# xinpw8/pokegym

Hardware: AMD Instinct MI355X
Metric: aggregate env.step/sec (higher is better)
Workload: dtype u8

## Files before the change

pokegym_amd/csrc/pk_capi.cpp:

```cpp
#include <hip/hip_runtime.h>

#include <errno.h>
#include <stdarg.h>
#include <stdio.h>
#include <stdlib.h>
#include <string.h>

#include <string>
#include <vector>

#include "../../include/pokegym_amd.h"
#include "pk_ucode.h"
#include "pk_layout.h"
#include "pk_reward.h"

hipError_t pk_launch_step(const PkStepArgs& a, hipStream_t s);
hipError_t pk_launch_step_small(const PkStepArgs& a, hipStream_t s);
hipError_t pk_launch_render(const PkStepArgs& a, hipStream_t s);
hipError_t pk_launch_reset(const PkResetArgs& a, hipStream_t s);
hipError_t pk_launch_list(const uint8_t* mask, uint32_t env0, uint32_t env1, uint32_t* cnt, uint32_t* ids, hipStream_t s);
hipError_t pk_launch_render_latched(const PkStepArgs& a, hipStream_t s);
hipError_t pk_launch_gather_env(const uint8_t* mem, uint32_t env, uint32_t sh, uint8_t* out, hipStream_t s);
hipError_t pk_launch_gather_range(const uint8_t* mem, uint32_t env0, uint32_t count, uint32_t sh, uint8_t* out, hipStream_t s);
hipError_t pk_launch_scatter_env(uint8_t* mem, uint32_t env, uint32_t sh, const uint8_t* in, hipStream_t s);
hipError_t pk_launch_done(const uint32_t* time_reg, uint32_t n, uint32_t max_steps, uint8_t* term,
                          uint8_t* trunc, double* rew, hipStream_t s);
hipError_t pk_launch_reward(const PkRewardArgs& a, hipStream_t s);
hipError_t pk_launch_rreset_pre(const PkRewardArgs& a, hipStream_t s);
hipError_t pk_launch_rreset_post(const PkRewardArgs& a, hipStream_t s);
hipError_t pk_launch_obs(const PkRewardArgs& a, hipStream_t s);
hipError_t pk_launch_seen_rehash(const uint32_t* old_tab, uint32_t old_lg, uint32_t* new_tab, uint32_t new_lg,
                                 const uint32_t* rs, uint32_t n, uint32_t np, hipStream_t s);
hipError_t pk_launch_ram_copy(uint8_t* mem, uint8_t* dense, uint32_t n, uint32_t sh, uint32_t phys0, uint32_t len,
                              uint32_t to_dense, hipStream_t s);
hipError_t pk_launch_bank_list(const PkBankArgs& a, hipStream_t s);
hipError_t pk_launch_bank_copy(const PkBankArgs& a, hipStream_t s);
hipError_t pk_launch_ep_move(const PkEpArgs& a, hipStream_t s);
hipError_t pk_launch_arch_update(const PkArchArgs& a, hipStream_t s);
hipError_t pk_launch_arch_draw(const PkArchArgs& a, hipStream_t s);
hipError_t pk_launch_arch_merge(const PkArchArgs& a, hipStream_t s);
hipError_t pk_launch_xchg_pack(const PkPackArgs& p, hipStream_t s);
hipError_t pk_launch_xchg_move(const PkXchgArgs& x, bool pack, hipStream_t s);
hipError_t pk_launch_arch_out(const PkArchArgs& a, hipStream_t s);
hipError_t pk_launch_cell_keys(const uint8_t* mem, uint32_t sh, uint32_t shift, uint64_t* keys, uint32_t env0,
                               uint32_t env1, hipStream_t s);
hipError_t pk_launch_frame_keys(const PkCellArgs& a, hipStream_t s);
hipError_t pk_launch_fstack(const PkStackArgs& a, hipStream_t s);
hipError_t pk_launch_cnt_update(const PkCountArgs& a, hipStream_t s);
hipError_t pk_launch_cnt_add(const PkCountArgs& a, hipStream_t s);
hipError_t pk_launch_cnt_pack(const PkCountArgs& a, hipStream_t s);
hipError_t pk_launch_traj_record(const PkTrajArgs& a, hipStream_t s);
hipError_t pk_launch_traj_reset(const PkTrajArgs& a, hipStream_t s);
hipError_t pk_launch_traj_mark(const PkTrajArgs& a, hipStream_t s);
hipError_t pk_launch_traj_move(const PkTrajArgs& a, hipStream_t s);
hipError_t pk_launch_traj_get(const PkTrajArgs& a, hipStream_t s);

namespace {

thread_local std::string g_err;

int fail(int code, const char* fmt, ...) {
    char buf[512];
    va_list ap;
    va_start(ap, fmt);
    vsnprintf(buf, sizeof buf, fmt, ap);
    va_end(ap);
    g_err = buf;
    return code;
}

#define HIPCHK(expr)                                                                       \
    do {                                                                                   \
        hipError_t e_ = (expr);                                                            \
        if (e_ != hipSuccess) return fail(-EIO, "%s: %s", #expr, hipGetErrorString(e_)); \
    } while (0)

constexpr size_t S_VER = 0, S_HDR = 1, S_CPU = 5, S_VRAM = 23, S_OAM = 8215, S_LCDREG = 8375,
                 S_LCDX = 8386, S_CLOCK = 8388, S_TARGET = 8396, S_NEXTMODE = 8404,
                 S_SCAN = 8405, S_SCREEN = 9125, S_WRAM = 101285, S_FEA0 = 109477,
                 S_IO = 109573, S_HRAM = 109649, S_FF4C = 109776, S_TIMER = 109828,
                 S_MBC = 109836, S_SRAM = 109842, S_SIZE = 142610;

struct Template {
    uint32_t regs[PK_NREGS];
    std::vector<uint8_t> mem;
    uint32_t lat[3 * PK_ROWS];
    std::vector<uint8_t> screen;
    uint8_t hdr[4];
    uint8_t lcdx[2];
};

uint64_t rd64(const uint8_t* p) {
    uint64_t v = 0;
    for (int i = 7; i >= 0; i--) v = (v << 8) | p[i];
    return v;
}
void wr64(uint8_t* p, uint64_t v) {
    for (int i = 0; i < 8; i++) { p[i] = (uint8_t)v; v >>= 8; }
}

int parse_v9(const uint8_t* s, size_t len, Template& t) {
// ... 608 lines not shown
    if (wram && (addr & 0x1FFF) + len > 0x2000) return fail(-EINVAL, "pk_set_ram: range wraps the echo mirror");
    HIPCHK(hipSetDevice(h->device));
    uint32_t phys0 = wram ? PK_P_WRAM + (addr & 0x1FFFu) : PK_P_HRAM + (addr - 0xFF80u);
    HIPCHK(pk_launch_ram_copy(h->mem, const_cast<uint8_t*>(dense), h->n, h->ilv_sh, phys0, len, 0, (hipStream_t)stream));
    return traj_mark(h, nullptr, nullptr, 0, h->n, (hipStream_t)stream);
}

static uint32_t k1_wave_lanes(const pk_handle* h, uint32_t count) {
    if (h->wave_lanes) return h->wave_lanes;
    const uint32_t npad = (count + PK_LANES - 1u) & ~(PK_LANES - 1u);
    if (npad / 64u >= 2u * h->simds) return 64u;
    if (npad / 32u >= 2u * h->simds) return 32u;
    if (npad / 16u > h->simds && npad / 16u <= 2u * h->simds) return 16u;
    return 32u;
}

static void k1_shape(const pk_handle* h, bool small, uint32_t& lanes, uint32_t& block, uint32_t& prio) {
    lanes = k1_wave_lanes(h, h->n);
    const uint32_t wg_envs = small ? PK_SMALL_WG_ENVS : PK_WG_ENVS;
    const uint32_t max_threads = small ? PK_SMALL_MAX_THREADS : PK_K1_MAX_THREADS;
    if (h->k1_block) {
        block = h->k1_block < max_threads ? h->k1_block : max_threads;
        if ((block / PK_LANES) * lanes > wg_envs) block = wg_envs / lanes * PK_LANES;
    } else {
        const uint32_t waves = ((h->n + PK_LANES - 1u) / PK_LANES) * (PK_LANES / lanes);
        const uint32_t wide = wg_envs * PK_LANES / lanes < max_threads ? wg_envs * PK_LANES / lanes : max_threads;
        block = waves <= h->simds ? 256u : wide;
    }
    prio = h->k1_prio >= 0 ? (uint32_t)h->k1_prio : (block > 256u && !small ? 1u : 0u);
}

static bool k1_small(const pk_handle* h, uint32_t env0, uint32_t env1) {
    if (h->k1_small >= 0) return h->k1_small != 0 && k1_wave_lanes(h, h->n) <= 32u;
    return (env1 - env0) < h->n && k1_wave_lanes(h, h->n) <= 32u;
}

static PkStepArgs step_args(pk_handle* h, const uint8_t* actions, uint32_t env0, uint32_t env1) {
    PkStepArgs a;
    memset(&a, 0, sizeof a);
    a.mem = h->mem; a.rom = h->rom; a.romw = reinterpret_cast<const uint32_t*>(h->rom); a.regs = h->regs; a.ucode = h->ucode; a.actions = actions;
    a.lat = h->lat; a.screen = h->screen; a.n = h->n; a.npad = h->npad;
    a.rom_bank_mask = h->bank_mask; a.mbc = h->mbc; a.frames = h->frames;
    a.release_frame = h->release; a.render_last = (h->flags & PK_F_RENDER) ? 1 : 0;
    a.lat_stride = (uint32_t)h->lat_stride;
    const bool small = k1_small(h, env0, env1);
    a.small = small ? 1u : 0u;
    a.nslots = small ? h->nslots_s : h->nslots;
    a.bank_slot = small ? h->bank_slot_s : h->bank_slot;
    a.slot_bank = small ? h->slot_bank_s : h->slot_bank;
    a.all_staged = a.nslots >= h->bank_mask + 1u ? 1u : 0u;
    k1_shape(h, small, a.wave_lanes, a.block, a.prio);
    a.simds = h->simds;
    a.dbg = h->dbg;
    a.env0 = env0; a.env1 = env1;
    a.ilv_sh = h->ilv_sh;
    return a;
}

int pk_render_latched(pk_handle* h, void* stream) {
    if (!h) return fail(-EINVAL, "null handle");
    HIPCHK(hipSetDevice(h->device));
    PkStepArgs a = step_args(h, nullptr, 0, h->n);
    HIPCHK(pk_launch_render_latched(a, (hipStream_t)stream));
    return 0;
}

int pk_step_range(pk_handle* h, uint32_t env0, uint32_t count, const uint8_t* actions, double* rew, uint8_t* term,
                  uint8_t* trunc, void* stream) {
    int rc;
    if ((rc = check_range(h, env0, count))) return rc;
    if (!actions) return fail(-EINVAL, "actions_dev is required");
    HIPCHK(hipSetDevice(h->device));
    hipStream_t s = (hipStream_t)stream;
    const uint32_t env1 = env0 + count;
    PkStepArgs a = step_args(h, actions, env0, env1);
    if (h->prof && (rc = prof_event(h, s))) return rc;
    HIPCHK(a.small ? pk_launch_step_small(a, s) : pk_launch_step(a, s));
    if (h->traj_cap) {
        PkTrajArgs t = traj_args(h, env0, env1);
        t.actions = actions;
        HIPCHK(pk_launch_traj_record(t, s));
    }
    if (h->prof && (rc = prof_event(h, s))) return rc;
    if (a.render_last) HIPCHK(pk_launch_render(a, s));
    if (h->prof && (rc = prof_event(h, s))) return rc;
    if (h->flags & PK_F_REWARD) {
        PkRewardArgs r = reward_args(h, env0, env1);
        r.actions = actions; r.rew = rew; r.term = term; r.trunc = trunc;
        HIPCHK(pk_launch_reward(r, s));
        HIPCHK(pk_launch_obs(r, s));
    } else if (rew || term || trunc) {
        HIPCHK(pk_launch_done(h->regs + (size_t)PK_R_TIME * h->npad + env0, count, h->max_steps, term ? term + env0 : nullptr,
                              trunc ? trunc + env0 : nullptr, rew ? rew + env0 : nullptr, s));
    }
    if (h->prof && (rc = prof_event(h, s))) return rc;
    return 0;
}

int pk_step(pk_handle* h, const uint8_t* actions, uint8_t* screen_out, double* rew, uint8_t* term,
            uint8_t* trunc, void* stream) {
    if (!h) return fail(-EINVAL, "null handle");
    int rc = pk_step_range(h, 0, h->n, actions, rew, term, trunc, stream);
    if (rc) return rc;
    if (screen_out)
        HIPCHK(hipMemcpyAsync(screen_out, h->screen, (size_t)h->n * PK_SCREEN, hipMemcpyDeviceToDevice, (hipStream_t)stream));
    return 0;
}

static int fetch_env(pk_handle* h, uint32_t env, std::vector<uint8_t>& mem, uint32_t* regs,
                     uint32_t* lat, std::vector<uint8_t>& screen) {
    if (env >= h->n) return fail(-EINVAL, "env %u out of range (n=%u)", env, h->n);
    HIPCHK(hipSetDevice(h->device));
    HIPCHK(hipDeviceSynchronize());
    HIPCHK(pk_launch_gather_env(h->mem, env, h->ilv_sh, h->scratch, nullptr));
    mem.resize(PK_PHYS);
    HIPCHK(hipMemcpy(mem.data(), h->scratch, PK_PHYS, hipMemcpyDeviceToHost));
    for (uint32_t f = 0; f < PK_NREGS; f++)
        HIPCHK(hipMemcpy(&regs[f], h->regs + (size_t)f * h->npad + env, 4, hipMemcpyDeviceToHost));
    uint32_t gid = env / PK_LANES, lane = env % PK_LANES;
    for (uint32_t k = 0; k < 3; k++) {
        std::vector<uint32_t> tmp((size_t)PK_ROWS * PK_LANES);
        HIPCHK(hipMemcpy(tmp.data(), h->lat + k * h->lat_stride + (size_t)gid * PK_ROWS * PK_LANES,
                         tmp.size() * 4, hipMemcpyDeviceToHost));
        for (uint32_t y = 0; y < PK_ROWS; y++) lat[k * PK_ROWS + y] = tmp[(size_t)y * PK_LANES + lane];
    }
    screen.resize(PK_SCREEN);
    HIPCHK(hipMemcpy(screen.data(), h->screen + (size_t)env * PK_SCREEN, PK_SCREEN, hipMemcpyDeviceToHost));
    return 0;
}

int pk_snapshot(pk_handle* h, uint32_t env, uint8_t* out, uint64_t len) {
    if (!h || !out) return fail(-EINVAL, "null argument");
    if (len < S_SIZE) return fail(-EINVAL, "buffer too small for a v9 state");
    std::vector<uint8_t> mem, screen;
    uint32_t regs[PK_NREGS], lat[3 * PK_ROWS];
    int rc = fetch_env(h, env, mem, regs, lat, screen);
    if (rc) return rc;
    export_v9(h->tmpl, regs, mem.data(), lat, screen.data(), out);
    return 0;
}

int pk_snapshot_range(pk_handle* h, uint32_t env0, uint32_t count, uint8_t* out, uint64_t len) {
    if (!h || !out) return fail(-EINVAL, "null argument");
    if (count == 0) return 0;
    if ((uint64_t)env0 + count > h->n) return fail(-EINVAL, "envs [%u, %u) out of range (n=%u)", env0, env0 + count, h->n);
    if (len < (uint64_t)count * S_SIZE) return fail(-EINVAL, "buffer too small for %u v9 states", count);
    HIPCHK(hipSetDevice(h->device));
    HIPCHK(hipDeviceSynchronize());
    const uint32_t chunk = count < 1024u ? count : 1024u;
    uint8_t* dmem = nullptr;
    HIPCHK(hipMalloc((void**)&dmem, (size_t)chunk * PK_PHYS));
    std::vector<uint8_t> mem((size_t)chunk * PK_PHYS), screen((size_t)chunk * PK_SCREEN);
    std::vector<uint32_t> regs((size_t)PK_NREGS * chunk), latg;
    int rc = 0;
    for (uint32_t c0 = 0; c0 < count && !rc; c0 += chunk) {
        const uint32_t e0 = env0 + c0, m = (count - c0) < chunk ? (count - c0) : chunk;
        hipError_t e = pk_launch_gather_range(h->mem, e0, m, h->ilv_sh, dmem, nullptr);
        if (e == hipSuccess) e = hipMemcpy(mem.data(), dmem, (size_t)m * PK_PHYS, hipMemcpyDeviceToHost);
        for (uint32_t f = 0; f < PK_NREGS && e == hipSuccess; f++)
            e = hipMemcpy(&regs[(size_t)f * chunk], h->regs + (size_t)f * h->npad + e0, (size_t)m * 4, hipMemcpyDeviceToHost);
        if (e == hipSuccess)
            e = hipMemcpy(screen.data(), h->screen + (size_t)e0 * PK_SCREEN, (size_t)m * PK_SCREEN, hipMemcpyDeviceToHost);
        const uint32_t g0 = e0 / PK_LANES, g1 = (e0 + m - 1) / PK_LANES + 1, rows = (g1 - g0) * PK_ROWS * PK_LANES;
        latg.resize((size_t)3 * rows);
        for (uint32_t k = 0; k < 3 && e == hipSuccess; k++)
            e = hipMemcpy(&latg[(size_t)k * rows], h->lat + k * h->lat_stride + (size_t)g0 * PK_ROWS * PK_LANES,
                          (size_t)rows * 4, hipMemcpyDeviceToHost);
        if (e != hipSuccess) { rc = fail(-EIO, "pk_snapshot_range: %s", hipGetErrorString(e)); break; }
        for (uint32_t i = 0; i < m; i++) {
            const uint32_t env = e0 + i, gi = env / PK_LANES - g0, lane = env % PK_LANES;
            uint32_t r[PK_NREGS], lat[3 * PK_ROWS];
            for (uint32_t f = 0; f < PK_NREGS; f++) r[f] = regs[(size_t)f * chunk + i];
            for (uint32_t k = 0; k < 3; k++)
                for (uint32_t y = 0; y < PK_ROWS; y++)
// ... 1091 lines not shown
```

pokegym_amd/csrc/pk_kernels.hip:

```cpp
#include <hip/hip_runtime.h>
#include <math.h>
#include <stdint.h>
#include <string.h>

#include "../../include/pokegym_amd.h"
#include "pk_layout.h"
#include "pk_render.h"

__global__ void __launch_bounds__(64) pk_render_kernel(PkStepArgs A) {
    const u32 y = blockIdx.x % PK_ROWS;
    const u32 gid = A.env0 / PK_LANES + blockIdx.x / PK_ROWS;
    const u32 lane = threadIdx.x;
    const u32 env = gid * PK_LANES + lane;
    if (env >= A.env1) return;
    const u32 rf = A.regs[PK_R_RFLAGS * A.npad + env];
    u8* out = A.screen + (size_t)env * PK_SCREEN + y * PK_COLS;
    const u32 idx = (gid * PK_ROWS + y) * PK_LANES + lane;
    const u32 l2 = A.lat[2u * A.lat_stride + idx];
    if (rf & 1u) {
        uint4 wv;
        wv.x = wv.y = wv.z = wv.w = 0xFFFFFFFFu;
        for (u32 q = 0; q < PK_COLS; q += 16) *reinterpret_cast<uint4*>(out + q) = wv;
        if (l2 & 0x100u) A.lat[2u * A.lat_stride + idx] = l2 & ~0x100u;
        return;
    }
    if (!(l2 & 0x100u)) return;
    const Mem m = mem_view(A.mem, env, A.ilv_sh);
    render_line(m, y, A.lat[idx], A.lat[A.lat_stride + idx], (int)(l2 & 0xFFu) - 1, out);
    A.lat[2u * A.lat_stride + idx] = l2 & ~0x100u;
}

__global__ void __launch_bounds__(256) pk_arm_latches_kernel(PkStepArgs A) {
    const u32 env = blockIdx.x * blockDim.x + threadIdx.x;
    if (env >= A.n) return;
    const u32 gid = env / PK_LANES, lane = env % PK_LANES;
    int lw = -1;
    for (u32 y = 0; y < PK_ROWS; y++) {
        const u32 idx = (gid * PK_ROWS + y) * PK_LANES + lane;
        const u32 l0 = A.lat[idx], l1 = A.lat[A.lat_stride + idx];
        const u32 wy = l1 & 0xFFu, wx = bfe8(l0, 24);
        if ((l0 & 0x20u) && wy <= y && (int)wx - 7 < (int)PK_COLS) lw += 1;
        A.lat[2u * A.lat_stride + idx] = (u32)(lw + 1) | 0x100u;
    }
    A.regs[PK_R_RFLAGS * A.npad + env] &= ~1u;
}



__global__ void __launch_bounds__(256) pk_list_kernel(const u8* mask, u32 env0, u32 env1, u32* cnt, u32* ids) {
    const u32 e = env0 + blockIdx.x * blockDim.x + threadIdx.x;
    if (e >= env1 || (mask && !mask[e])) return;
    ids[atomicAdd(cnt, 1u)] = e;
}

__global__ void __launch_bounds__(256) pk_reset_mem_kernel(PkResetArgs A) {
    const u32 cnt = *A.cnt;
    for (u32 k = threadIdx.x; k < cnt; k += blockDim.x) {
        const u32 env = A.ids[k];
        const Mem m = mem_view(A.mem, env, A.ilv_sh);
        for (u32 p = blockIdx.x; p < PK_PHYS; p += gridDim.x) st_phys(m, p, A.tmpl_mem[p]);
    }
}

__global__ void __launch_bounds__(256) pk_reset_regs_kernel(PkResetArgs A) {
    const u32 cnt = *A.cnt;
    for (u32 k = blockIdx.x * blockDim.x + threadIdx.x; k < cnt; k += gridDim.x * blockDim.x) {
        const u32 env = A.ids[k];
        for (u32 f = 0; f < PK_NREGS; f++) A.regs[f * A.npad + env] = A.tmpl_regs[f];
        const u32 gid = env / PK_LANES, lane = env % PK_LANES;
        for (u32 j = 0; j < 3u; j++)
            for (u32 y = 0; y < PK_ROWS; y++)
                A.lat[j * A.lat_stride + (gid * PK_ROWS + y) * PK_LANES + lane] = A.tmpl_lat[j * PK_ROWS + y];
        const uint4* s = reinterpret_cast<const uint4*>(A.tmpl_screen);
        uint4* d = reinterpret_cast<uint4*>(A.screen + (size_t)env * PK_SCREEN);
        for (u32 q = 0; q < PK_SCREEN / 16u; q++) d[q] = s[q];
    }
}

__global__ void pk_gather_env_kernel(const u8* mem, u32 env, u32 sh, u8* out) {
    const Mem m = mem_view(const_cast<u8*>(mem), env, sh);
    for (u32 p = blockIdx.x * blockDim.x + threadIdx.x; p < PK_PHYS; p += gridDim.x * blockDim.x)
        out[p] = ld_phys(m, p);
}

__global__ void __launch_bounds__(256) pk_gather_range_kernel(const u8* mem, u32 env0, u32 count, u32 sh, u8* out) {
    const size_t total = (size_t)count * PK_PHYS;
    for (size_t t = (size_t)blockIdx.x * blockDim.x + threadIdx.x; t < total; t += (size_t)gridDim.x * blockDim.x) {
        const u32 k = (u32)(t % count), p = (u32)(t / count);
        const u32 env = env0 + k;
        out[(size_t)k * PK_PHYS + p] = mem[pk_img_off(env, p, sh)];
    }
}

__global__ void pk_scatter_env_kernel(u8* mem, u32 env, u32 sh, const u8* in) {
    const Mem m = mem_view(mem, env, sh);
    for (u32 p = blockIdx.x * blockDim.x + threadIdx.x; p < PK_PHYS; p += gridDim.x * blockDim.x)
        st_phys(m, p, in[p]);
}

hipError_t pk_launch_render(const PkStepArgs& a, hipStream_t s) {
    const u32 grid = ((a.env1 - a.env0 + PK_LANES - 1u) / PK_LANES) * PK_ROWS;
    hipLaunchKernelGGL(pk_render_kernel, dim3(grid), dim3(PK_LANES), 0, s, a);
    return hipGetLastError();
}

hipError_t pk_launch_render_latched(const PkStepArgs& a, hipStream_t s) {
    hipLaunchKernelGGL(pk_arm_latches_kernel, dim3((a.env1 + 255) / 256), dim3(256), 0, s, a);
    hipError_t e = hipGetLastError();
    if (e != hipSuccess) return e;
    return pk_launch_render(a, s);
}

hipError_t pk_launch_list(const u8* mask, u32 env0, u32 env1, u32* cnt, u32* ids, hipStream_t s) {
    hipLaunchKernelGGL(pk_list_kernel, dim3((env1 - env0 + 255) / 256), dim3(256), 0, s, mask, env0, env1, cnt, ids);
    return hipGetLastError();
}

hipError_t pk_launch_reset(const PkResetArgs& a, hipStream_t s) {
    hipLaunchKernelGGL(pk_reset_mem_kernel, dim3(4096), dim3(256), 0, s, a);
    hipError_t e = hipGetLastError();
    if (e != hipSuccess) return e;
    hipLaunchKernelGGL(pk_reset_regs_kernel, dim3((a.env1 - a.env0 + 255) / 256), dim3(256), 0, s, a);
    return hipGetLastError();
}

hipError_t pk_launch_gather_env(const u8* mem, u32 env, u32 sh, u8* out, hipStream_t s) {
    hipLaunchKernelGGL(pk_gather_env_kernel, dim3(64), dim3(256), 0, s, mem, env, sh, out);
    return hipGetLastError();
}

hipError_t pk_launch_gather_range(const u8* mem, u32 env0, u32 count, u32 sh, u8* out, hipStream_t s) {
    hipLaunchKernelGGL(pk_gather_range_kernel, dim3(2048), dim3(256), 0, s, mem, env0, count, sh, out);
    return hipGetLastError();
}

hipError_t pk_launch_scatter_env(u8* mem, u32 env, u32 sh, const u8* in, hipStream_t s) {
    hipLaunchKernelGGL(pk_scatter_env_kernel, dim3(64), dim3(256), 0, s, mem, env, sh, in);
    return hipGetLastError();
}

__global__ void pk_done_kernel(const u32* time_reg, u32 n, u32 max_steps, u8* term, u8* trunc, double* rew) {
    const u32 e = blockIdx.x * blockDim.x + threadIdx.x;
    if (e >= n) return;
    const u8 done = time_reg[e] >= max_steps ? 1 : 0;
    if (term) term[e] = done;
    if (trunc) trunc[e] = done;
    if (rew) rew[e] = 0.0;
}

hipError_t pk_launch_done(const u32* time_reg, u32 n, u32 max_steps, u8* term, u8* trunc, double* rew, hipStream_t s) {
    hipLaunchKernelGGL(pk_done_kernel, dim3((n + 255) / 256), dim3(256), 0, s, time_reg, n, max_steps, term, trunc, rew);
    return hipGetLastError();
}


__global__ void __launch_bounds__(256) pk_bank_list_kernel(PkBankArgs A) {
    const u32 e = A.env0 + blockIdx.x * blockDim.x + threadIdx.x;
    if (e >= A.env1) return;
    int32_t s = -1;
    bool tmpl = false;
    if (A.mode != PK_BANK_RESET || !A.sel || A.sel[e]) {
        s = A.slot_of_env[e];
        if (s < 0) {
            s = -1;
            tmpl = A.mode == PK_BANK_RESET;
        } else if ((u32)s >= A.n_slots || (A.mode != PK_BANK_SAVE && !A.b_filled[s]) ||
                   (A.mode == PK_BANK_LOAD && A.ep && !A.b_ep_filled[s])) {
            atomicAdd(A.b_rejects, 1u);
            s = -1;
            tmpl = A.mode == PK_BANK_RESET;
        }
    }
    A.src[e] = s;
    if (s >= 0) A.ids[atomicAdd(A.cnt, 1u)] = e;
    if (tmpl) A.tids[atomicAdd(A.tcnt, 1u)] = e;
}

__global__ void __launch_bounds__(256) pk_bank_subs_kernel(PkBankArgs A) {
    const u32 sb = (A.env0 >> A.ilv_sh) + blockIdx.x * blockDim.x + threadIdx.x;
    const u32 e0 = sb << A.ilv_sh;
    for (u32 j = 0; j < (1u << A.ilv_sh); j++)
        if (e0 + j < A.env1 && A.src[e0 + j] >= 0) {
            A.subs[atomicAdd(A.cnt + 1, 1u)] = sb;
            return;
        }
}
// ... 1044 lines not shown
```

pokegym_amd/csrc/pk_layout.h:

```cpp
#pragma once
#include <hip/hip_runtime.h>
#include <stdint.h>

typedef struct { uint32_t x, y; } uint2_t;

#define PK_LANES 64u
#define PK_PHYS 0xC200u
#ifndef PK_SKEW
#define PK_SKEW 0u
#endif
#define PK_GROUP_STRIDE (PK_PHYS * PK_LANES + PK_SKEW * PK_LANES)

__host__ __device__ static inline uint64_t pk_sub_stride(uint32_t sh) { return ((uint64_t)PK_PHYS << sh) + PK_SKEW; }
__host__ __device__ static inline uint64_t pk_group_stride(uint32_t sh) { return (uint64_t)(PK_LANES >> sh) * pk_sub_stride(sh); }

__host__ __device__ static inline uint64_t pk_img_off(uint32_t env, uint32_t phys, uint32_t sh) {
    const uint32_t l = env & (PK_LANES - 1u);
    return (uint64_t)(env / PK_LANES) * pk_group_stride(sh) + (uint64_t)(l >> sh) * pk_sub_stride(sh)
         + ((uint64_t)phys << sh) + (l & ((1u << sh) - 1u));
}

#define PK_P_VRAM 0x0000u
#define PK_P_WRAM 0x2000u
#define PK_P_OAM 0x4000u
#define PK_P_IO 0x4100u
#define PK_P_HRAM 0x4180u
#define PK_P_SRAM 0x4200u
#define PK_P_UNUSED 0x41FFu

#define PK_ROWS 144u
#define PK_COLS 160u
#define PK_SCREEN (PK_ROWS * PK_COLS)

enum {
    PK_R_W0 = 0,
    PK_R_W1,
    PK_R_SP,
    PK_R_PC,
    PK_R_CPU,
    PK_R_CLOCK,
    PK_R_TARGET,
    PK_R_LCD0,
    PK_R_LCD1,
    PK_R_LCD2,
    PK_R_TIM0,
    PK_R_TIM1,
    PK_R_MBC,
    PK_R_MISC,
    PK_R_TIME,
    PK_R_ICOUNT,
    PK_R_RFLAGS,
    PK_NREGS
};

#ifdef PK_WAVETIME
#define PK_WT_REC 6u
#define PK_DBG_WORDS (64u + PK_WT_REC * 16384u)
#else
#define PK_DBG_WORDS 64u
#endif

#define PK_SMALL_LDS_SLOTS 2u
#define PK_SMALL_WG_ENVS 128u
#define PK_SMALL_MAX_THREADS 256
#ifdef PK_K1_SMALL
#define PK_WG_ENVS PK_SMALL_WG_ENVS
#define PK_LDS_SLOTS PK_SMALL_LDS_SLOTS
#define PK_K1_MAX_THREADS PK_SMALL_MAX_THREADS
#endif
#ifndef PK_K1_MAX_THREADS
#define PK_K1_MAX_THREADS 512
#endif
#ifndef PK_WG_ENVS
#define PK_WG_ENVS 512u
#endif
#ifndef PK_LDS_SLOTS
#define PK_LDS_SLOTS 6u
#endif

struct PkStepArgs {
    uint8_t* mem;
    const uint8_t* rom;
    const uint32_t* romw;
    uint32_t* regs;
    const uint32_t* ucode;
    const uint8_t* actions;
    uint32_t* lat;
    uint8_t* screen;
    uint32_t n, npad;
    uint32_t rom_bank_mask;
    uint32_t mbc;
    uint32_t frames;
    uint32_t release_frame;
    uint32_t render_last;
    uint32_t lat_stride;
    uint32_t nslots;
    const int8_t* bank_slot;
    const uint8_t* slot_bank;
    uint32_t wave_lanes;
    uint32_t simds;
    uint32_t block;
    uint32_t prio;
    unsigned long long* dbg;
    uint32_t env0, env1;
    uint32_t ilv_sh;
    uint32_t small;
    uint32_t all_staged;
};

struct PkResetArgs {
    uint8_t* mem;
    uint32_t* regs;
    uint32_t* lat;
    uint8_t* screen;
    const uint8_t* tmpl_mem;
    const uint32_t* tmpl_regs;
    const uint32_t* tmpl_lat;
    const uint8_t* tmpl_screen;
    const uint32_t* cnt;
    const uint32_t* ids;
    uint32_t n, npad, lat_stride;
    uint32_t env0, env1;
    uint32_t ilv_sh;
};

#define PK_BANK_REGS 20u
#define PK_BANK_MAX_SLOTS 65536u
#define PK_BANK_TILE 16384u
enum { PK_BANK_LOAD = 0, PK_BANK_SAVE = 1, PK_BANK_RESET = 2 };

struct PkBankArgs {
    uint8_t* mem;
    uint32_t* regs;
    uint32_t* lat;
    uint8_t* screen;
    uint8_t* b_mem;
    uint32_t* b_regs;
    uint32_t* b_lat;
    uint8_t* b_screen;
    uint8_t* b_filled;
    uint8_t* b_ep_filled;
    uint32_t* b_rejects;
    const int32_t* slot_of_env;
    const uint8_t* sel;
    int32_t* src;
    uint32_t* cnt;
    uint32_t* ids;
    uint32_t* subs;
    uint32_t* tcnt;
    uint32_t* tids;
    uint32_t n_slots;
    uint32_t mode;
    uint32_t ep;
    uint32_t n, npad, lat_stride;
    uint32_t env0, env1;
    uint32_t ilv_sh;
};

#define PK_ARCH_MAX_CELLS 65536u
#define PK_ARCH_NOKEY 0xFFFFFFFFFFFFFFFFull
#define PK_ARCH_NONE 0xFFFFFFFFu
#define PK_ARCH_PRE 8u
enum { PK_AH_USED = 0, PK_AH_OVERFLOW, PK_AH_DRAWS, PK_AH_CUR, PK_AH_TOTAL, PK_AH_WORDS = 8 };

struct PkArchArgs {
    uint64_t* hdr;
    uint64_t* a_key;
    double* a_score;
    uint32_t* a_len;
    uint32_t* a_visits;
    uint32_t* a_picks;
    uint64_t* prefix;
    uint64_t* i_key;
    uint32_t* i_cell;
    uint64_t* c_max;
    uint64_t* c_le;
    uint64_t* s_key;
    uint64_t* s_max;
    uint64_t* s_le;
    uint32_t* s_first;
    uint32_t* s_cnt;
    uint32_t* s_cell;
    uint32_t* tgt;
    uint8_t* flag;
    int32_t* map;
    const uint64_t* keys;
    const double* scores;
    const uint8_t* mask;
    const uint32_t* time_reg;
    uint32_t* b_rejects;
// ... 100 lines not shown
```

pokegym_amd/csrc/pk_render.h:

```cpp
#pragma once
#include <hip/hip_runtime.h>
#include <stdint.h>

#include "pk_layout.h"

typedef uint32_t u32;
typedef uint8_t u8;

__device__ __forceinline__ u32 bfe8(u32 v, u32 sh) { return (v >> sh) & 0xFFu; }
__device__ __forceinline__ u32 setb8(u32 v, u32 sh, u32 b) { return (v & ~(0xFFu << sh)) | ((b & 0xFFu) << sh); }

struct Mem {
    u8* g;
    u32 lane;
    u32 sh;
};
__device__ __forceinline__ u32 ld_phys(const Mem& m, u32 phys) { return m.g[(phys << m.sh) + m.lane]; }
__device__ __forceinline__ void st_phys(const Mem& m, u32 phys, u32 v) { m.g[(phys << m.sh) + m.lane] = (u8)v; }
__device__ __forceinline__ Mem mem_view(u8* mem, u32 env, u32 sh) {
    Mem m;
    m.g = mem + pk_img_off(env, 0u, sh) - (env & (PK_LANES - 1u) & ((1u << sh) - 1u));
    m.lane = env & (PK_LANES - 1u) & ((1u << sh) - 1u);
    m.sh = sh;
    return m;
// ... 21 lines not shown
        int run;
        if (win && wx <= x) {
            int wxx = x - wx;
            u32 t = ld_phys(m, PK_P_VRAM + wmap + (u32)(((lw / 8) * 32) % 0x400) + (u32)((wxx / 8) % 32));
            u32 ta = bg_tile_addr(lcdc, t) + (u32)(lw % 8) * 2u;
            lo = ld_phys(m, PK_P_VRAM + ta);
            hi = ld_phys(m, PK_P_VRAM + ta + 1u);
            sub = (u32)(wxx % 8);
            run = 8 - (int)sub;
        } else if (lcdc & 0x01u) {
            int xx = x + bx;
            u32 t = ld_phys(m, PK_P_VRAM + bgmap + (u32)((((y + (u32)by) / 8u) * 32u) % 0x400u) + (u32)((xx / 8) % 32));
            u32 ta = bg_tile_addr(lcdc, t) + ((y + (u32)by) % 8u) * 2u;
            lo = ld_phys(m, PK_P_VRAM + ta);
            hi = ld_phys(m, PK_P_VRAM + ta + 1u);
            sub = (u32)(xx % 8);
            run = 8 - (int)sub;
            if (win && wx > x && wx < x + run) run = wx - x;
        } else {
            line[x] = 0;
            x++;
            continue;
        }
        for (int k = 0; k < run && x < (int)PK_COLS; k++, x++) {
            u32 s = 7u - (sub + (u32)k);
            u32 ci = ((lo >> s) & 1u) | (((hi >> s) & 1u) << 1);
            line[x] = (u8)((bgp >> (2u * ci)) & 3u);
        }
    }
    if (lcdc & 0x02u) {
        int h = (lcdc & 0x04u) ? 16 : 8;
        int sel[10];
        int ns = 0;
        for (int n = 0; n < 40 && ns < 10; n++) {
            int sy = (int)ld_phys(m, PK_P_OAM + (u32)n * 4u) - 16;
            if (sy <= (int)y && (int)y < sy + h) sel[ns++] = n;
        }
        for (int i = 1; i < ns; i++) {
            int k = sel[i], j = i - 1;
            u32 kx = ld_phys(m, PK_P_OAM + (u32)k * 4u + 1u);
            while (j >= 0 && ld_phys(m, PK_P_OAM + (u32)sel[j] * 4u + 1u) > kx) { sel[j + 1] = sel[j]; j--; }
            sel[j + 1] = k;
        }
        u32 bg0 = bgp & 3u;
        for (int i = ns - 1; i >= 0; i--) {
            u32 base = PK_P_OAM + (u32)sel[i] * 4u;
            int sy = (int)ld_phys(m, base) - 16, sx = (int)ld_phys(m, base + 1u) - 8;
            u32 ti = ld_phys(m, base + 2u), at = ld_phys(m, base + 3u);
            if (h == 16) ti &= 0xFEu;
            int dy = (int)y - sy;
            int yy = (at & 0x40u) ? (h - dy - 1) : dy;
            u32 pal = (at & 0x10u) ? obp1 : obp0;
            u32 ta = ti * 16u + (u32)yy * 2u;
            u32 lo = ld_phys(m, PK_P_VRAM + ta), hi = ld_phys(m, PK_P_VRAM + ta + 1u);
            for (int dx = 0; dx < 8; dx++) {
                int px = sx + dx;
                u32 xx = (at & 0x20u) ? (u32)(7 - dx) : (u32)dx;
                u32 s = 7u - xx;
                u32 c = ((lo >> s) & 1u) | (((hi >> s) & 1u) << 1);
                if (px >= 0 && px < (int)PK_COLS && c != 0u) {
                    u32 shade = (pal >> (2u * c)) & 3u;
                    if (at & 0x80u) {
                        if (line[px] == bg0) line[px] = (u8)shade;
                    } else {
                        line[px] = (u8)shade;
                    }
                }
            }
        }
    }
    for (int q = 0; q < (int)PK_COLS; q += 16) {
        uint4 v;
        u32 w[4];
        for (int j = 0; j < 4; j++) {
            u32 a = 0;
            for (int b = 0; b < 4; b++) a |= grey(line[q + j * 4 + b]) << (8 * b);
            w[j] = a;
        }
        v.x = w[0]; v.y = w[1]; v.z = w[2]; v.w = w[3];
        *reinterpret_cast<uint4*>(out + q) = v;
    }
}

#ifndef PK_FLUSH_STAT
#define PK_FLUSH_STAT(rendered) ((void)0)
#endif

__device__ __forceinline__ u32 pend_add(u32 p, u32 lo, u32 hi) {
    const u32 h1 = hi + 1u;
    return p == 0u ? (h1 | (lo << 16)) : ((((p & 0xFFFFu) > h1) ? (p & 0xFFFFu) : h1) | (((p >> 16) < lo ? (p >> 16) : lo) << 16));
}

__device__ __noinline__ static void flush_lines(u32* lat, u32 lat_stride, u8* screen, u8* gbase, u32 il, u32 sh, u32 lane,
                                                u32 env, u32 gid, u32 pend) {
    Mem m;
    m.g = gbase;
    m.lane = il;
    m.sh = sh;
    u32* lat0 = lat;
    u32* lat1 = lat + lat_stride;
    u32* lat2 = lat + 2u * lat_stride;
#ifndef PK_FLUSH_FULL
    const u32 ylo = pend >> 16, yend = pend & 0xFFFFu;
#else
    const u32 ylo = 0u, yend = pend ? PK_ROWS : 0u;
#endif
    for (u32 y0 = ylo; y0 < yend; y0 += 16u) {
        u32 f[16];
#pragma unroll
        for (u32 k = 0; k < 16u; k++) {
            const u32 y = y0 + k < PK_ROWS ? y0 + k : PK_ROWS - 1u;
            f[k] = lat2[(gid * PK_ROWS + y) * PK_LANES + lane];
        }
        for (u32 k = 0; k < 16u && y0 + k < yend; k++) {
            const u32 y = y0 + k, idx = (gid * PK_ROWS + y) * PK_LANES + lane, l2 = f[k];
            if (l2 & 0x100u) {
                render_line(m, y, lat0[idx], lat1[idx], (int)(l2 & 0xFFu) - 1, screen + (size_t)env * PK_SCREEN + y * PK_COLS);
                lat2[idx] = l2 & ~0x100u;
                PK_FLUSH_STAT(1);
            }
        }
    }
    PK_FLUSH_STAT(0);
}
```

Before: 1.005 million.

## Render scanlines with bitplane register math and fuse done flags into render

Replaces the per-pixel scanline renderer in the render kernel with a bit-sliced version. Tile rows and sprites are packed into 32-bit plane words and combined with alignbit, bit-select and perm operations. Sprite ordering uses a register sorting network instead of an insertion sort that rereads OAM. When rewards are off and done outputs are requested, the term/trunc/rew writes are folded into the render kernel to save a launch. The trade-off is more register pressure from the unrolled arrays and more complexity around pixel accuracy for edge cases such as sprite priority and window masking.

```diff
diff --git a/pokegym_amd/csrc/pk_capi.cpp b/pokegym_amd/csrc/pk_capi.cpp
--- a/pokegym_amd/csrc/pk_capi.cpp
+++ b/pokegym_amd/csrc/pk_capi.cpp
@@ -17,6 +17,7 @@
 hipError_t pk_launch_step(const PkStepArgs& a, hipStream_t s);
 hipError_t pk_launch_step_small(const PkStepArgs& a, hipStream_t s);
 hipError_t pk_launch_render(const PkStepArgs& a, hipStream_t s);
+hipError_t pk_launch_render_done(const PkStepArgs& a, const PkDoneArgs& d, hipStream_t s);
 hipError_t pk_launch_reset(const PkResetArgs& a, hipStream_t s);
 hipError_t pk_launch_list(const uint8_t* mask, uint32_t env0, uint32_t env1, uint32_t* cnt, uint32_t* ids, hipStream_t s);
 hipError_t pk_launch_render_latched(const PkStepArgs& a, hipStream_t s);
@@ -791,14 +792,23 @@
         HIPCHK(pk_launch_traj_record(t, s));
     }
     if (h->prof && (rc = prof_event(h, s))) return rc;
-    if (a.render_last) HIPCHK(pk_launch_render(a, s));
+    const bool fuse_done = a.render_last && !(h->flags & PK_F_REWARD) && (rew || term || trunc);
+    if (fuse_done) {
+        PkDoneArgs d;
+        d.time_reg = h->regs + (size_t)PK_R_TIME * h->npad;
+        d.term = term; d.trunc = trunc; d.rew = rew;
+        d.max_steps = h->max_steps; d.on = 1u;
+        HIPCHK(pk_launch_render_done(a, d, s));
+    } else if (a.render_last) {
+        HIPCHK(pk_launch_render(a, s));
+    }
     if (h->prof && (rc = prof_event(h, s))) return rc;
     if (h->flags & PK_F_REWARD) {
         PkRewardArgs r = reward_args(h, env0, env1);
         r.actions = actions; r.rew = rew; r.term = term; r.trunc = trunc;
         HIPCHK(pk_launch_reward(r, s));
         HIPCHK(pk_launch_obs(r, s));
-    } else if (rew || term || trunc) {
+    } else if (!fuse_done && (rew || term || trunc)) {
         HIPCHK(pk_launch_done(h->regs + (size_t)PK_R_TIME * h->npad + env0, count, h->max_steps, term ? term + env0 : nullptr,
                               trunc ? trunc + env0 : nullptr, rew ? rew + env0 : nullptr, s));
     }
diff --git a/pokegym_amd/csrc/pk_kernels.hip b/pokegym_amd/csrc/pk_kernels.hip
--- a/pokegym_amd/csrc/pk_kernels.hip
+++ b/pokegym_amd/csrc/pk_kernels.hip
@@ -7,12 +7,18 @@
 #include "pk_layout.h"
 #include "pk_render.h"
 
-__global__ void __launch_bounds__(64) pk_render_kernel(PkStepArgs A) {
+__global__ void __launch_bounds__(64) pk_render_kernel(PkStepArgs A, PkDoneArgs D) {
     const u32 y = blockIdx.x % PK_ROWS;
     const u32 gid = A.env0 / PK_LANES + blockIdx.x / PK_ROWS;
     const u32 lane = threadIdx.x;
     const u32 env = gid * PK_LANES + lane;
     if (env >= A.env1) return;
+    if (D.on && y == 0u) {
+        const u8 done = D.time_reg[env] >= D.max_steps ? 1 : 0;
+        if (D.term) D.term[env] = done;
+        if (D.trunc) D.trunc[env] = done;
+        if (D.rew) D.rew[env] = 0.0;
+    }
     const u32 rf = A.regs[PK_R_RFLAGS * A.npad + env];
     u8* out = A.screen + (size_t)env * PK_SCREEN + y * PK_COLS;
     const u32 idx = (gid * PK_ROWS + y) * PK_LANES + lane;
@@ -25,8 +31,8 @@
         return;
     }
     if (!(l2 & 0x100u)) return;
-    const Mem m = mem_view(A.mem, env, A.ilv_sh);
-    render_line(m, y, A.lat[idx], A.lat[A.lat_stride + idx], (int)(l2 & 0xFFu) - 1, out);
+    const MemW m = memw_view(A.mem, gid, lane, A.ilv_sh);
+    render_line_regs(m, y, A.lat[idx], A.lat[A.lat_stride + idx], (int)(l2 & 0xFFu) - 1, out);
     A.lat[2u * A.lat_stride + idx] = l2 & ~0x100u;
 }
 
@@ -98,10 +104,16 @@
         st_phys(m, p, in[p]);
 }
 
+hipError_t pk_launch_render_done(const PkStepArgs& a, const PkDoneArgs& d, hipStream_t s) {
+    const u32 grid = ((a.env1 - a.env0 + PK_LANES - 1u) / PK_LANES) * PK_ROWS;
+    hipLaunchKernelGGL(pk_render_kernel, dim3(grid), dim3(PK_LANES), 0, s, a, d);
+    return hipGetLastError();
+}
+
 hipError_t pk_launch_render(const PkStepArgs& a, hipStream_t s) {
-    const u32 grid = ((a.env1 - a.env0 + PK_LANES - 1u) / PK_LANES) * PK_ROWS;
-    hipLaunchKernelGGL(pk_render_kernel, dim3(grid), dim3(PK_LANES), 0, s, a);
-    return hipGetLastError();
+    PkDoneArgs d;
+    memset(&d, 0, sizeof d);
+    return pk_launch_render_done(a, d, s);
 }
 
 hipError_t pk_launch_render_latched(const PkStepArgs& a, hipStream_t s) {
diff --git a/pokegym_amd/csrc/pk_layout.h b/pokegym_amd/csrc/pk_layout.h
--- a/pokegym_amd/csrc/pk_layout.h
+++ b/pokegym_amd/csrc/pk_layout.h
@@ -106,6 +106,15 @@
     uint32_t ilv_sh;
     uint32_t small;
     uint32_t all_staged;
+};
+
+struct PkDoneArgs {
+    const uint32_t* time_reg;
+    uint8_t* term;
+    uint8_t* trunc;
+    double* rew;
+    uint32_t max_steps;
+    uint32_t on;
 };
 
 struct PkResetArgs {
diff --git a/pokegym_amd/csrc/pk_render.h b/pokegym_amd/csrc/pk_render.h
--- a/pokegym_amd/csrc/pk_render.h
+++ b/pokegym_amd/csrc/pk_render.h
@@ -127,6 +127,190 @@
     }
 }
 
+#ifdef __HIPCC__
+__device__ __forceinline__ u32 pk_alignbit(u32 hi, u32 lo, u32 sh) { return __builtin_amdgcn_alignbit(hi, lo, sh); }
+__device__ __forceinline__ u32 pk_brev32(u32 v) { return __builtin_bitreverse32(v); }
+#else
+static inline u32 pk_alignbit(u32 hi, u32 lo, u32 sh) { return (u32)((((uint64_t)hi << 32) | lo) >> (sh & 31u)); }
+static inline u32 pk_brev32(u32 v) {
+    v = ((v >> 1) & 0x55555555u) | ((v & 0x55555555u) << 1);
+    v = ((v >> 2) & 0x33333333u) | ((v & 0x33333333u) << 2);
+    v = ((v >> 4) & 0x0F0F0F0Fu) | ((v & 0x0F0F0F0Fu) << 4);
+    return (v >> 24) | ((v >> 8) & 0xFF00u) | ((v << 8) & 0xFF0000u) | (v << 24);
+}
+#endif
+__device__ __forceinline__ u32 bsel(u32 mask, u32 a, u32 b) { return (a & mask) | (b & ~mask); }
+__device__ __forceinline__ u32 bit_fill(u32 v, u32 k) { return 0u - ((v >> k) & 1u); }
+
+struct MemW {
+    const u8* gb;
+    u32 lo;
+    u32 sh;
+};
+__device__ __forceinline__ u32 ldw(const MemW& m, u32 phys) { return m.gb[m.lo + (phys << m.sh)]; }
+__device__ __forceinline__ MemW memw_view(const u8* mem, u32 gid, u32 l, u32 sh) {
+    MemW m;
+    m.gb = mem + (uint64_t)gid * pk_group_stride(sh);
+    m.lo = (l >> sh) * (u32)pk_sub_stride(sh) + (l & ((1u << sh) - 1u));
+    m.sh = sh;
+    return m;
+}
+
+__device__ __forceinline__ void tile_planes(const MemW& m, u32 maprow, u32 c0, u32 lcdc, u32 fine, bool last,
+                                            u32 (&pl)[6], u32 (&ph)[6]) {
+    const u32 flip = (lcdc & 0x10u) ? 0u : 0x80u;
+    const u32 base = PK_P_VRAM + ((lcdc & 0x10u) ? 0u : 0x800u) + fine * 2u;
+    u32 t[21], lo[24], hi[24];
+#pragma unroll
+    for (u32 k = 0; k < 21u; k++) t[k] = (k < 20u || last) ? ldw(m, maprow + ((c0 + k) & 31u)) : 0u;
+#pragma unroll
+    for (u32 k = 0; k < 24u; k++) {
+        lo[k] = hi[k] = 0u;
+        if (k < 20u || (k == 20u && last)) {
+            const u32 ta = base + ((t[k] ^ flip) << 4);
+            lo[k] = ldw(m, ta);
+            hi[k] = ldw(m, ta + 1u);
+        }
+    }
+#pragma unroll
+    for (u32 i = 0; i < 6u; i++) {
+        const u32 a = lo[4 * i] | (lo[4 * i + 1] << 8) | (lo[4 * i + 2] << 16) | (lo[4 * i + 3] << 24);
+        const u32 b = hi[4 * i] | (hi[4 * i + 1] << 8) | (hi[4 * i + 2] << 16) | (hi[4 * i + 3] << 24);
+        pl[i] = __builtin_amdgcn_perm(0u, pk_brev32(a), 0x00010203u);
+        ph[i] = __builtin_amdgcn_perm(0u, pk_brev32(b), 0x00010203u);
+    }
+}
+
+#define PK_OBJ_LINE 10
+
+__device__ __forceinline__ void render_line_regs(const MemW& m, u32 y, u32 lat0, u32 lat1, int lw, u8* out) {
+    const u32 lcdc = lat0 & 0xFFu;
+    const u32 bx = bfe8(lat0, 8), by = bfe8(lat0, 16);
+    const int wx = (int)bfe8(lat0, 24) - 7, wy = (int)(lat1 & 0xFFu);
+    const u32 bgp = bfe8(lat1, 8), obp0 = bfe8(lat1, 16), obp1 = bfe8(lat1, 24);
+    const bool win = (lcdc & 0x20u) && wy <= (int)y && wx < (int)PK_COLS;
+    const bool bgon = (lcdc & 0x01u) != 0u;
+    u32 c0[5], c1[5];
+#pragma unroll
+    for (u32 i = 0; i < 5u; i++) c0[i] = c1[i] = 0u;
+    if (bgon && !(win && wx <= 0)) {
+        const u32 yy = y + by, fs = bx & 7u;
+        u32 pl[6], ph[6];
+        tile_planes(m, PK_P_VRAM + ((lcdc & 0x08u) ? 0x1C00u : 0x1800u) + ((yy >> 3) & 31u) * 32u, bx >> 3, lcdc, yy & 7u,
+                    fs != 0u, pl, ph);
+#pragma unroll
+        for (u32 i = 0; i < 5u; i++) {
+            c0[i] = pk_alignbit(pl[i + 1], pl[i], fs);
+            c1[i] = pk_alignbit(ph[i + 1], ph[i], fs);
+        }
+    }
+    u32 wm[5];
+#pragma unroll
+    for (u32 i = 0; i < 5u; i++) wm[i] = 0u;
+    if (win) {
+        const u32 lwu = (u32)lw & 0xFFu, nwx = (u32)(-wx), fs = nwx & 7u;
+        u32 pl[6], ph[6];
+        tile_planes(m, PK_P_VRAM + ((lcdc & 0x40u) ? 0x1C00u : 0x1800u) + ((lwu >> 3) & 31u) * 32u, (u32)((int)nwx >> 3), lcdc,
+                    lwu & 7u, fs != 0u, pl, ph);
+#pragma unroll
+        for (u32 i = 0; i < 5u; i++) {
+            int n = wx - (int)(32u * i);
+            n = n < 0 ? 0 : (n > 32 ? 32 : n);
+            wm[i] = (0xFFFFFFFFu << ((u32)n >> 1)) << ((u32)n - ((u32)n >> 1));
+            c0[i] = bsel(wm[i], pk_alignbit(pl[i + 1], pl[i], fs), c0[i]);
+            c1[i] = bsel(wm[i], pk_alignbit(ph[i + 1], ph[i], fs), c1[i]);
+        }
+    }
+    u32 s0[5], s1[5];
+    {
+        const u32 p00 = bit_fill(bgp, 0), p01 = bit_fill(bgp, 1), p10 = bit_fill(bgp, 2), p11 = bit_fill(bgp, 3);
+        const u32 p20 = bit_fill(bgp, 4), p21 = bit_fill(bgp, 5), p30 = bit_fill(bgp, 6), p31 = bit_fill(bgp, 7);
+        const u32 keep = bgon ? 0xFFFFFFFFu : 0u;
+#pragma unroll
+        for (u32 i = 0; i < 5u; i++) {
+            s0[i] = bsel(c1[i], bsel(c0[i], p30, p20), bsel(c0[i], p10, p00)) & (wm[i] | keep);
+            s1[i] = bsel(c1[i], bsel(c0[i], p31, p21), bsel(c0[i], p11, p01)) & (wm[i] | keep);
+        }
+    }
+    if (lcdc & 0x02u) {
+        const u32 h = (lcdc & 0x04u) ? 16u : 8u;
+        u32 K[PK_OBJ_LINE];
+#pragma unroll
+        for (u32 i = 0; i < PK_OBJ_LINE; i++) K[i] = 0u;
+        u32 ns = 0;
+#pragma unroll
+        for (u32 n0 = 0; n0 < 40u; n0 += 10u) {
+            u32 oy[10], ox[10];
+#pragma unroll
+            for (u32 k = 0; k < 10u; k++) {
+                oy[k] = ldw(m, PK_P_OAM + (n0 + k) * 4u);
+                ox[k] = ldw(m, PK_P_OAM + (n0 + k) * 4u + 1u);
+            }
+#pragma unroll
+            for (u32 k = 0; k < 10u; k++) {
+                if (y + 16u - oy[k] < h && ns < PK_OBJ_LINE) {
+                    ns++;
+                    u32 key = (ox[k] << 16) | ((n0 + k) << 8) | oy[k];
+#pragma unroll
+                    for (u32 i = 0; i < PK_OBJ_LINE; i++) {
+                        const u32 a = K[i];
+                        K[i] = a > key ? a : key;
+                        key = a > key ? key : a;
+                    }
+                }
+            }
+        }
+        const u32 b0 = bit_fill(bgp, 0), b1 = bit_fill(bgp, 1);
+        while (K[0] != 0u) {
+            const u32 key = K[0];
+#pragma unroll
+            for (u32 i = 0; i + 1u < PK_OBJ_LINE; i++) K[i] = K[i + 1];
+            K[PK_OBJ_LINE - 1] = 0u;
+            const u32 base = PK_P_OAM + ((key >> 8) & 0xFFu) * 4u;
+            u32 ti = ldw(m, base + 2u);
+            const u32 at = ldw(m, base + 3u);
+            if (h == 16u) ti &= 0xFEu;
+            const u32 dy = y + 16u - (key & 0xFFu);
+            const u32 yy = (at & 0x40u) ? (h - 1u - dy) : dy;
+            const u32 ta = PK_P_VRAM + ti * 16u + yy * 2u;
+            const u32 w = ldw(m, ta) | (ldw(m, ta + 1u) << 8);
+            const u32 r = pk_brev32(w);
+            const u32 ol = (at & 0x20u) ? (w & 0xFFu) : (r >> 24), oh = (at & 0x20u) ? (w >> 8) : ((r >> 16) & 0xFFu);
+            const u32 pal = (at & 0x10u) ? obp1 : obp0;
+            const u32 om = ol | oh;
+            const u32 v0 = bsel(oh, bsel(ol, bit_fill(pal, 6), bit_fill(pal, 4)), ol & bit_fill(pal, 2)) & om;
+            const u32 v1 = bsel(oh, bsel(ol, bit_fill(pal, 7), bit_fill(pal, 5)), ol & bit_fill(pal, 3)) & om;
+            const u32 pos = (key >> 16) + 24u, j0 = pos >> 5, sft = pos & 31u;
+            const u32 mlo = om << sft, mhi = (om >> 1) >> (31u - sft);
+            const u32 v0lo = v0 << sft, v0hi = (v0 >> 1) >> (31u - sft);
+            const u32 v1lo = v1 << sft, v1hi = (v1 >> 1) >> (31u - sft);
+            const u32 front = (at & 0x80u) ? 0u : 0xFFFFFFFFu;
+#pragma unroll
+            for (u32 i = 0; i < 5u; i++) {
+                const bool isl = j0 == i + 1u, ish = j0 == i;
+                u32 mk = isl ? mlo : (ish ? mhi : 0u);
+                mk &= front | ~((s0[i] ^ b0) | (s1[i] ^ b1));
+                s0[i] = bsel(mk, isl ? v0lo : v0hi, s0[i]);
+                s1[i] = bsel(mk, isl ? v1lo : v1hi, s1[i]);
+            }
+        }
+    }
+#pragma unroll
+    for (u32 q = 0; q < PK_COLS / 16u; q++) {
+        u32 wv[4];
+#pragma unroll
+        for (u32 j = 0; j < 4u; j++) {
+            const u32 sft = (q & 1u) * 16u + j * 4u;
+            const u32 l4 = (s0[q >> 1] >> sft) & 15u, h4 = (s1[q >> 1] >> sft) & 15u;
+            const u32 sel = ((l4 * 0x00204081u) & 0x01010101u) | (((h4 * 0x00204081u) & 0x01010101u) << 1);
+            wv[j] = __builtin_amdgcn_perm(0u, 0x005599FFu, sel);
+        }
+        uint4 v;
+        v.x = wv[0]; v.y = wv[1]; v.z = wv[2]; v.w = wv[3];
+        *reinterpret_cast<uint4*>(out + q * 16u) = v;
+    }
+}
+
 #ifndef PK_FLUSH_STAT
 #define PK_FLUSH_STAT(rendered) ((void)0)
 #endif
```

Result: faster. 1.019 million, median of 6 (+1.3%).
